# apple/ml-4m

Measured on AMD Instinct MI355X. Metric: multimodal tokens/sec (4M-B train step, whole job), higher is better.
Workload: dtype bf16; 1 GPU; 4M-B mod7 (fm_base_12e_12d_swiglu_nobias, 360.8M params, 8 input / 7 target modalities) masked-modeling train step, 224^2 token grids, 128 input + 128 target tokens/sample, AdamW; model=fm_base_12e_12d_swiglu_nobias, per_gpu_batch=256, global_batch=256, seq_len=256, parallelism=dp1

## Files before the change

### include/fourm_hip.h

```cpp
#ifndef FOURM_HIP_H
#define FOURM_HIP_H
#include <stdint.h>

#ifdef __cplusplus
extern "C" {
#endif

#define FM_ABI_VERSION 11
int fm_abi_version(void);
const char* fm_last_error(void);

enum fm_epilogue {
    FM_EPI_BF16 = 0,
    FM_EPI_GELU = 1,
    FM_EPI_RESIDUAL = 2,
    FM_EPI_SWIGLU = 3,
    FM_EPI_F32 = 4,
    FM_EPI_TANH = 5,
    FM_EPI_SWIGLU_BWD = 6,
    FM_EPI_GELU_BWD = 7,
    FM_EPI_QUICK_GELU = 8,
    FM_EPI_RELU = 9,
    FM_EPI_RELU_BWD = 10
};
// ... 158 lines not shown
} fm_embed_bwd_desc;
int fm_embed_bwd(const fm_embed_bwd_desc* desc, void* stream);

int fm_dense_decoder_mask(const int32_t* cs, const int16_t* mod, void* out, int B, int M, int causal, int use_cs,
                          int use_sep, void* stream);

enum fm_loss_type { FM_LOSS_MOD = 0, FM_LOSS_TOKEN = 1 };
#define FM_SEG_ROWS 256
int fm_segment_rows(const int32_t* head_of_row, int R, int n_heads, int32_t* seg_start, int32_t* seg_count,
                    int32_t* perm, int32_t* row_to_padded, int32_t* tile_group, int Rp, void* stream);
int fm_gather_rows(const void* src, int ld_src, const int32_t* perm, void* dst, int ld_dst, int Rp, int D, void* stream);
int fm_cross_entropy(void* logits, int ldl, const int32_t* perm, const int32_t* tile_group, const int64_t* target_ids,
                     const int32_t* vocab, const int32_t* seg_start, const int32_t* seg_count, const void* grad_scale,
                     int loss_type, int n_heads, int Rp, int max_vocab, void* row_loss, void* row_lse, void* head_loss,
                     void* total_loss, int write_grad, void* stream);

int fm_swiglu_bwd(const void* da, int ldda, const void* gu, int ldgu, void* dgu, int lddgu, int R, int H, int Hp, void* stream);
int fm_gelu_bwd(const void* dh, int lddh, const void* pre, int ldp, void* dpre, int lddp, int R, int H, int Hp, void* stream);
typedef struct fm_shadow_desc {
    const void* src; void* dst;
    int32_t ld_src, ld_dst, rows, cols, transpose, tile_start;
    const void* col_scale;
    int32_t dst_f32, reserved;
} fm_shadow_desc;
int fm_shadow_refresh(const fm_shadow_desc* descs, int n_descs, int total_tiles, void* stream);
#define FM_FOLD_MAX_JOBS 48
typedef struct fm_fold_grad_job {
    const void* dWp; const void* W; const void* gamma; void* gW; void* ggamma;
    int32_t rows, cols, ld_dwp, reserved;
} fm_fold_grad_job;
// ... 223 lines not shown
```

### ml-4m_amd/csrc/loss.hip

```cpp
#include "common.h"
#include "fourm_hip.h"

namespace {

constexpr int SEG_ALIGN = FM_SEG_ROWS;

__global__ __launch_bounds__(1024) void segment_rows_kernel(const int32_t* __restrict__ head_of_row, int R, int n_heads,
                                                            int32_t* __restrict__ seg_start, int32_t* __restrict__ seg_count,
                                                            int32_t* __restrict__ perm, int32_t* __restrict__ row_to_padded,
                                                            int32_t* __restrict__ tile_group, int Rp) {
    __shared__ int cnt[FM_MAX_MODS];
    __shared__ int wtot[16];
    const int g = blockIdx.x, tid = threadIdx.x, lane = tid & 63, wave = tid >> 6;
    if (tid < FM_MAX_MODS) cnt[tid] = 0;
    __syncthreads();
    for (int r = tid; r < R; r += 1024) {
        const int hh = head_of_row[r];
        if (hh >= 0 && hh <= g) atomicAdd(&cnt[hh], 1);
    }
    __syncthreads();
    int start = 0;
    for (int m = 0; m < g; ++m) start += (cnt[m] + SEG_ALIGN - 1) / SEG_ALIGN * SEG_ALIGN;
    const int mine = cnt[g];
    const int padded = (mine + SEG_ALIGN - 1) / SEG_ALIGN * SEG_ALIGN;
// ... 22 lines not shown
        run += tot;
    }
}

__global__ void fill_i32_kernel(int32_t* p, int v, int n) {
    const int i = blockIdx.x * 256 + threadIdx.x;
    if (i < n) p[i] = v;
}

__device__ __forceinline__ void online_merge(float& m, float& s, float m2, float s2) {
    const float mn = fmaxf(m, m2);
    s = s * __expf(m - mn) + s2 * __expf(m2 - mn);
    m = mn;
}

__global__ __launch_bounds__(256) void ce_fwd_kernel(const bf16_t* __restrict__ logits, int ldl, const int32_t* __restrict__ perm,
                                                     const int32_t* __restrict__ tile_group, const long long* __restrict__ target_ids,
                                                     const int32_t* __restrict__ vocab, float* __restrict__ row_loss, float* __restrict__ row_lse) {
    __shared__ float red_m[4], red_s[4];
    const int pr = blockIdx.x;
    const int g = tile_group[pr / SEG_ALIGN];
    if (g < 0) return;
    const int src = perm[pr];
    if (src < 0) {
        if (threadIdx.x == 0) { row_loss[pr] = 0.f; row_lse[pr] = 0.f; }
        return;
    }
    const int V = vocab[g];
    const bf16_t* row = logits + (size_t)pr * ldl;
    float m = -INFINITY, ssum = 0.f;
    for (int c = threadIdx.x * 8; c < V; c += 256 * 8) {
        float v[8];
        if (c + 8 <= V) {
            const uint4 p = *(const uint4*)(row + c);
            const uint32_t w[4] = {p.x, p.y, p.z, p.w};
#pragma unroll
            for (int e = 0; e < 4; ++e) { v[2 * e] = bf2f((bf16_t)(w[e] & 0xffff)); v[2 * e + 1] = bf2f((bf16_t)(w[e] >> 16)); }
        } else {
#pragma unroll
            for (int e = 0; e < 8; ++e) v[e] = c + e < V ? bf2f(row[c + e]) : -INFINITY;
        }
        float cm = v[0];
#pragma unroll
        for (int e = 1; e < 8; ++e) cm = fmaxf(cm, v[e]);
        const float mn = fmaxf(m, cm);
        float add = 0.f;
#pragma unroll
        for (int e = 0; e < 8; ++e) add += __expf(v[e] - mn);
        ssum = ssum * __expf(m - mn) + add;
        m = mn;
    }
#pragma unroll
    for (int o = 32; o > 0; o >>= 1) {
        const float m2 = __shfl_xor(m, o, 64), s2 = __shfl_xor(ssum, o, 64);
        if (m2 > -INFINITY || m > -INFINITY) online_merge(m, ssum, m2, s2);
    }
    const int lane = threadIdx.x & 63, wave = threadIdx.x >> 6;
    if (lane == 0) { red_m[wave] = m; red_s[wave] = ssum; }
    __syncthreads();
    if (threadIdx.x == 0) {
        float M = red_m[0], S = red_s[0];
        for (int w = 1; w < 4; ++w)
            if (red_m[w] > -INFINITY) online_merge(M, S, red_m[w], red_s[w]);
        const float lse = M + __logf(S);
        row_lse[pr] = lse;
        row_loss[pr] = lse - bf2f(row[target_ids[src]]);
    }
}

__global__ __launch_bounds__(256) void ce_bwd_kernel(bf16_t* __restrict__ logits, int ldl, const int32_t* __restrict__ perm,
                                                     const int32_t* __restrict__ tile_group, const long long* __restrict__ target_ids,
                                                     const int32_t* __restrict__ vocab, const int32_t* __restrict__ seg_count,
                                                     const float* __restrict__ gscale, int loss_type, int n_heads,
                                                     const float* __restrict__ row_lse) {
    const int pr = blockIdx.x;
    const int g = tile_group[pr / SEG_ALIGN];
    if (g < 0) return;
    const int V = vocab[g];
    const int Vp = (V + 63) / 64 * 64;
    bf16_t* row = logits + (size_t)pr * ldl;
    const int src = perm[pr];
    if (src < 0) {
        for (int c = threadIdx.x; c < Vp / 8; c += 256) *(uint4*)(row + c * 8) = make_uint4(0u, 0u, 0u, 0u);
        return;
    }
    float w;
    if (loss_type == FM_LOSS_MOD) {
        w = 1.0f / ((float)seg_count[g] * (float)n_heads);
    } else {
        float tot = 0.f;
        for (int mm = 0; mm < n_heads; ++mm) tot += (float)seg_count[mm] * (float)vocab[mm];
        w = (float)V / tot;
    }
    w *= gscale ? gscale[0] : 1.0f;
    const float lse = row_lse[pr];
    const int tgt = (int)target_ids[src];
    for (int c = threadIdx.x * 8; c < Vp; c += 256 * 8) {
        const uint4 p = *(const uint4*)(row + c);
        const uint32_t wd[4] = {p.x, p.y, p.z, p.w};
        float o[8];
#pragma unroll
        for (int e = 0; e < 8; ++e) {
            const float x = bf2f((bf16_t)((e & 1) ? (wd[e >> 1] >> 16) : (wd[e >> 1] & 0xffff)));
            o[e] = (c + e < V) ? (__expf(x - lse) - ((c + e) == tgt ? 1.f : 0.f)) * w : 0.f;
        }
        *(uint4*)(row + c) = make_uint4(pack2bf(o[0], o[1]), pack2bf(o[2], o[3]), pack2bf(o[4], o[5]), pack2bf(o[6], o[7]));
    }
}

__global__ __launch_bounds__(256) void loss_finalize_kernel(const float* __restrict__ row_loss, const int32_t* __restrict__ seg_start,
                                                            const int32_t* __restrict__ seg_count, const int32_t* __restrict__ vocab,
                                                            int n_heads, int loss_type, float* __restrict__ head_loss, float* __restrict__ total) {
    __shared__ float red[4];
    __shared__ float hl[FM_MAX_MODS];
    const int lane = threadIdx.x & 63, wave = threadIdx.x >> 6;
    for (int g = 0; g < n_heads; ++g) {
        const int s0 = seg_start[g], n = seg_count[g];
        float s = 0.f;
        for (int i = threadIdx.x; i < n; i += 256) s += row_loss[s0 + i];
        s = wave_sum(s);
        if (lane == 0) red[wave] = s;
// ... 11 lines not shown
        total[0] = tot / wsum;
    }
}

__global__ __launch_bounds__(256) void ce_f32_kernel(float* logits, int ld, const int* perm, const int* tile_group, const long long* target_ids,
                                                     const int* vocab, const int* seg_count, const float* grad_scale, int loss_type, int n_heads,
                                                     float* row_loss, float* row_lse, int write_grad, int seg_rows) {
    __shared__ float red[4];
    const int pr = blockIdx.x;
    const int g = tile_group[pr / seg_rows];
    if (g < 0) return;
    const int src = perm[pr];
    const int V = vocab[g];
    float* row = logits + (size_t)pr * ld;
    if (src < 0) {
        if (!write_grad) { if (threadIdx.x == 0) { row_loss[pr] = 0.f; row_lse[pr] = 0.f; } }
        else for (int c = threadIdx.x; c < V; c += 256) row[c] = 0.f;
        return;
    }
    const int tgt = (int)target_ids[src];
    if (!write_grad) {
        float mx = -INFINITY;
        for (int c = threadIdx.x; c < V; c += 256) mx = fmaxf(mx, row[c]);
        mx = wave_max(mx);
        __syncthreads();
        if ((threadIdx.x & 63) == 0) red[threadIdx.x >> 6] = mx;
        __syncthreads();
        mx = fmaxf(fmaxf(red[0], red[1]), fmaxf(red[2], red[3]));
        float s = 0.f;
        for (int c = threadIdx.x; c < V; c += 256) s += expf(row[c] - mx);
        s = wave_sum(s);
        __syncthreads();
        if ((threadIdx.x & 63) == 0) red[threadIdx.x >> 6] = s;
        __syncthreads();
        s = (red[0] + red[1]) + (red[2] + red[3]);
        const float lse = mx + logf(s);
        if (threadIdx.x == 0) { row_lse[pr] = lse; row_loss[pr] = lse - row[tgt]; }
        return;
    }
    float coef;
    if (loss_type == FM_LOSS_MOD) coef = 1.0f / ((float)n_heads * (float)seg_count[g]);
    else {
        double tot = 0.0;
        for (int h = 0; h < n_heads; ++h) tot += (double)seg_count[h] * (double)vocab[h];
        coef = (float)((double)V / tot);
    }
    coef *= grad_scale ? grad_scale[0] : 1.0f;
    const float lse = row_lse[pr];
    for (int c = threadIdx.x; c < V; c += 256) row[c] = coef * (expf(row[c] - lse) - (c == tgt ? 1.0f : 0.f));
}


__global__ __launch_bounds__(256) void gather_rows_kernel(const bf16_t* __restrict__ src, int lds_, const int32_t* __restrict__ perm,
                                                          bf16_t* __restrict__ dst, int ldd, int Rp, int D) {
    const int lane = threadIdx.x & 63, wave = threadIdx.x >> 6;
    for (int pr = blockIdx.x * 4 + wave; pr < Rp; pr += gridDim.x * 4) {
        const int s = perm[pr];
        for (int c = lane; c < D / 8; c += 64) {
            uint4 v = make_uint4(0u, 0u, 0u, 0u);
            if (s >= 0) v = *(const uint4*)(src + (size_t)s * lds_ + c * 8);
            *(uint4*)(dst + (size_t)pr * ldd + c * 8) = v;
        }
    }
// ... 20 lines not shown
    if (grid > 4096) grid = 4096;
    hipLaunchKernelGGL(gather_rows_kernel, dim3(grid), dim3(256), 0, (hipStream_t)stream, (const bf16_t*)src, ld_src, perm, (bf16_t*)dst, ld_dst, Rp, D);
    FM_CHECK_LAUNCH("fm_gather_rows");
    return 0;
}

extern "C" int fm_cross_entropy(void* logits, int ldl, const int32_t* perm, const int32_t* tile_group, const int64_t* target_ids,
                                const int32_t* vocab, const int32_t* seg_start, const int32_t* seg_count, const void* grad_scale,
                                int loss_type, int n_heads, int Rp, int max_vocab, void* row_loss, void* row_lse, void* head_loss,
                                void* total_loss, int write_grad, void* stream) {
    FM_CHECK_ARG(logits && perm && tile_group && target_ids && vocab && seg_start && seg_count && row_loss && row_lse && head_loss && total_loss,
                 "fm_cross_entropy: null pointer");
    FM_CHECK_ARG(loss_type == FM_LOSS_MOD || loss_type == FM_LOSS_TOKEN, "fm_cross_entropy: invalid loss type %d", loss_type);
    FM_CHECK_ARG(ldl % 8 == 0 && ldl >= (max_vocab + 63) / 64 * 64, "fm_cross_entropy: ldl=%d too small for vocab %d", ldl, max_vocab);
    FM_CHECK_ARG((((uintptr_t)logits) & 15) == 0, "fm_cross_entropy: logits must be 16-byte aligned");
    if (!write_grad) {
        hipLaunchKernelGGL(ce_fwd_kernel, dim3(Rp), dim3(256), 0, (hipStream_t)stream, (const bf16_t*)logits, ldl, perm, tile_group,
                           (const long long*)target_ids, vocab, (float*)row_loss, (float*)row_lse);
        hipLaunchKernelGGL(loss_finalize_kernel, dim3(1), dim3(256), 0, (hipStream_t)stream, (const float*)row_loss, seg_start, seg_count,
                           vocab, n_heads, loss_type, (float*)head_loss, (float*)total_loss);
    } else {
        hipLaunchKernelGGL(ce_bwd_kernel, dim3(Rp), dim3(256), 0, (hipStream_t)stream, (bf16_t*)logits, ldl, perm, tile_group,
                           (const long long*)target_ids, vocab, seg_count, (const float*)grad_scale, loss_type, n_heads, (const float*)row_lse);
    }
    FM_CHECK_LAUNCH("fm_cross_entropy");
    return 0;
}

extern "C" int fm_cross_entropy_f32(void* logits, int ldl, const int32_t* perm, const int32_t* tile_group, const int64_t* target_ids,
                                    const int32_t* vocab, const int32_t* seg_start, const int32_t* seg_count, const void* grad_scale,
                                    int loss_type, int n_heads, int Rp, int max_vocab, void* row_loss, void* row_lse, void* head_loss,
                                    void* total_loss, int write_grad, void* stream) {
    FM_CHECK_ARG(logits && perm && tile_group && target_ids && vocab && seg_start && seg_count && row_loss && row_lse && head_loss && total_loss,
                 "fm_cross_entropy_f32: null pointer");
    FM_CHECK_ARG(loss_type == FM_LOSS_MOD || loss_type == FM_LOSS_TOKEN, "fm_cross_entropy_f32: invalid loss type %d", loss_type);
    FM_CHECK_ARG(ldl >= max_vocab, "fm_cross_entropy_f32: ldl=%d too small for vocab %d", ldl, max_vocab);
    hipLaunchKernelGGL(ce_f32_kernel, dim3(Rp), dim3(256), 0, (hipStream_t)stream, (float*)logits, ldl, perm, tile_group,
                       (const long long*)target_ids, vocab, seg_count, (const float*)grad_scale, loss_type, n_heads, (float*)row_loss,
                       (float*)row_lse, write_grad, SEG_ALIGN);
    if (!write_grad)
        hipLaunchKernelGGL(loss_finalize_kernel, dim3(1), dim3(256), 0, (hipStream_t)stream, (const float*)row_loss, seg_start, seg_count,
                           vocab, n_heads, loss_type, (float*)head_loss, (float*)total_loss);
    FM_CHECK_LAUNCH("fm_cross_entropy_f32");
    return 0;
}
```

### ml-4m_amd/fourm/hip/_lib.py

```python
import ctypes as C
import os

FM_MAX_MODS = 24
_LIB_PATH = os.environ.get("FOURM_HIP_LIB") or os.path.join(os.path.dirname(os.path.dirname(os.path.abspath(__file__))), "_lib", "libfourm_hip.so")


class FourmHipUnavailable(ImportError):
    pass


def _load():
    if not os.path.exists(_LIB_PATH):
        raise FourmHipUnavailable(
            f"{_LIB_PATH} is missing - build the gfx950 kernels first: python ml-4m_amd/build_ext.py "
            "(the 4M hot path has no fallback implementation)")
    return C.CDLL(_LIB_PATH)


lib = _load()
lib.fm_last_error.restype = C.c_char_p
lib.fm_abi_version.restype = C.c_int
ABI_VERSION = 11
if lib.fm_abi_version() != ABI_VERSION:
    raise FourmHipUnavailable(f"libfourm_hip.so ABI {lib.fm_abi_version()} != expected {ABI_VERSION}; rebuild")
# ... 129 lines not shown
gemm_tn_multi = _sig("fm_gemm_tn_multi", P(GemmTNJob), C.c_int, vp)
layernorm_fwd = _sig("fm_layernorm_fwd", vp, i32, vp, vp, vp, i32, i32, vp, vp, vp, i32, i32, f32, vp)
layernorm_fwd_res = _sig("fm_layernorm_fwd_res", vp, i32, vp, i32, vp, i32, vp, vp, vp, i32, i32, vp, vp, vp, i32, i32, f32, vp)
layernorm_bwd = _sig("fm_layernorm_bwd", vp, i32, vp, vp, i32, vp, vp, vp, vp, vp, i32, vp, i32, vp, vp, i32, i32, vp)
layernorm_bwd_h = _sig("fm_layernorm_bwd_h", vp, i32, vp, i32, vp, i32, vp, vp, vp, vp, vp, i32, vp, i32, vp, i32, i32, vp)
attn_fwd = _sig("fm_attn_fwd", P(AttnArgs), vp)
attn_bwd = _sig("fm_attn_bwd", P(AttnArgs), vp)
attn_decode = _sig("fm_attn_decode", P(AttnDecodeArgs), vp)
ATTN_DECODE_MAX_NK = 8192
select_embed = _sig("fm_select_embed", P(SelectDesc), vp)
embed_bwd = _sig("fm_embed_bwd", P(EmbedBwdDesc), vp)
dense_decoder_mask = _sig("fm_dense_decoder_mask", vp, vp, vp, i32, i32, i32, i32, i32, vp)
segment_rows = _sig("fm_segment_rows", vp, i32, i32, vp, vp, vp, vp, vp, i32, vp)
gather_rows = _sig("fm_gather_rows", vp, i32, vp, vp, i32, i32, i32, vp)
cross_entropy = _sig("fm_cross_entropy", vp, i32, vp, vp, vp, vp, vp, vp, vp, i32, i32, i32, i32, vp, vp, vp, vp, i32, vp)
swiglu_bwd = _sig("fm_swiglu_bwd", vp, i32, vp, i32, vp, i32, i32, i32, i32, vp)
gelu_bwd = _sig("fm_gelu_bwd", vp, i32, vp, i32, vp, i32, i32, i32, i32, vp)
cast_pad = _sig("fm_cast_pad", vp, i32, vp, i32, i32, i32, vp)
transpose_cast_pad = _sig("fm_transpose_cast_pad", vp, i32, vp, i32, i32, i32, i32, vp)
colsum = _sig("fm_colsum", vp, i32, vp, i32, i32, vp)
shadow_refresh = _sig("fm_shadow_refresh", vp, i32, i32, vp)
fold_colscale_grad = _sig("fm_fold_colscale_grad", vp, i32, vp)
headnorm_fwd = _sig("fm_headnorm_fwd", vp, i32, vp, vp, vp, i32, vp, i32, i32, C.c_float, vp)
headnorm_bwd = _sig("fm_headnorm_bwd", vp, i32, vp, i32, vp, vp, vp, i32, vp, vp, i32, i32, vp)
f32_to_bf16 = _sig("fm_f32_to_bf16", vp, vp, i64, vp)
bf16_to_f32_scaled = _sig("fm_bf16_to_f32_scaled", vp, vp, i64, f32, vp)
add_bf16_f32 = _sig("fm_add_bf16_f32", vp, vp, vp, i64, vp)
lib.fm_set_reserved_cus.argtypes = [C.c_int]
lib.fm_get_reserved_cus.restype = C.c_int
lib.fm_get_reserved_cus.argtypes = []
# ... 103 lines not shown
ssim_scale_scratch = _sig("fm_ssim_scale_scratch", i32, i32, i32, i32, i32)
ssim_scale = _sig("fm_ssim_scale", vp, vp, i32, i32, i32, i32, i32, i32, i32, vp, i32, f32, f32, vp, vp, vp, vp)
avgpool2x2_pair = _sig("fm_avgpool2x2_pair", vp, vp, i32, i32, i32, i32, i32, i32, i32, vp, vp, vp)
token_histogram = _sig("fm_token_histogram", vp, i32, i64, i32, vp, vp, vp)
RESIZE_BILINEAR, RESIZE_BILINEAR_AA, RESIZE_NEAREST = 0, 1, 2
RESIZE_MAX_TAPS = 64
resize_axis_table = _sig("fm_resize_axis_table", i32, i32, i32, P(i32), P(i32), P(f32), P(C.c_double), P(i32), P(i32))
resize_bilinear_fwd = _sig("fm_resize_bilinear_fwd", vp, vp, i32, i32, i32, i32, i32, vp, vp, vp, i32, vp, vp, vp, i32, vp, vp, i32, vp)
resize_bilinear_bwd = _sig("fm_resize_bilinear_bwd", vp, vp, i32, i32, i32, i32, i32, vp, vp, vp, i32, vp, vp, vp, vp, vp, i32, vp, vp, vp, i32, vp)
resize_nearest = _sig("fm_resize_nearest", vp, vp, i32, i32, i32, i32, i32, i32, vp, vp, vp)
EXPORTS = ["fm_resize_axis_table", "fm_resize_bilinear_fwd", "fm_resize_bilinear_bwd", "fm_resize_nearest","fm_metric_sums_scratch", "fm_metric_sums", "fm_ssim_scale_scratch", "fm_ssim_scale", "fm_avgpool2x2_pair", "fm_token_histogram",
           "fm_reconst_loss_scratch", "fm_reconst_loss", "fm_scale_f32", "fm_mask_out_samples", "fm_ema_update", "fm_diffusion_pair", "fm_token_usage", "fm_lpips_stem", "fm_lpips_stem_bwd", "fm_maxpool2x2_nhwc", "fm_lpips_distance", "fm_lpips_tap_bwd", "fm_feat_distance", "fm_quick_gelu_bwd", "fm_quick_gelu_bwd_f32", "fm_clip_embed_ln_bwd", "fm_tap_add", "fm_clip_embed_ln", "fm_attn_decode", "fm_vit_patch_rows", "fm_vit_emb_rows", "fm_vit_colsum", "fm_lora_apply", "fm_lora_grad", "fm_vq_assign_wide", "fm_memcodes_assign", "fm_convnext_block", "fm_split3_bf16", "fm_unet_im2col", "fm_groupnorm_nhwc", "fm_add_bf16", "fm_silu_f32_to_bf16", "fm_timestep_embedding", "fm_unet_attention", "fm_diffusion_x0", "fm_quantile_abs",
           "fm_diffusion_step", "fm_unpack_image_u8", "fm_unpack_ids_u16", "fm_unpack_mask_bits", "fm_decoder_attention_from_target", "fm_guidance_combine", "fm_image_mask", "fm_token_budgets", "fm_span_mask", "fm_vq_code_stats", "fm_vq_ema_update", "fm_vq_code_bias", "fm_vq_assign_bias", "fm_vq_code_stats_raw", "fm_vq_ema_update_euclid", "fm_vq_unpatchify", "fm_vq_latent_grad", "fm_tanh_bwd_f32", "fm_embed_rows_f32", "fm_vq_patchify_ex", "fm_vq_cls_emb_bwd", "fm_vq_latent_grad_normalized", "fm_abi_version", "fm_last_error", "fm_gemm_nt", "fm_set_gemm_nt_config", "fm_get_gemm_nt_config", "fm_set_reserved_cus", "fm_get_reserved_cus", "fm_bf16_to_f32_scaled", "fm_add_bf16_f32", "fm_scale_rows_bf16", "fm_gemm_tn", "fm_gemm_tn_multi", "fm_set_gemm_tn_config", "fm_get_gemm_tn_config", "fm_set_tn_transpose_read",
           "fm_get_tn_transpose_read", "fm_layernorm_fwd", "fm_layernorm_fwd_res", "fm_layernorm_bwd", "fm_layernorm_bwd_h", "fm_headnorm_fwd", "fm_headnorm_bwd", "fm_attn_fwd", "fm_attn_bwd",
           "fm_set_attn_transpose_read", "fm_get_attn_transpose_read", "fm_select_embed", "fm_embed_bwd",
           "fm_dense_decoder_mask", "fm_segment_rows", "fm_gather_rows", "fm_cross_entropy", "fm_swiglu_bwd",
           "fm_gelu_bwd", "fm_cast_pad", "fm_transpose_cast_pad", "fm_shadow_refresh", "fm_fold_colscale_grad", "fm_colsum", "fm_f32_to_bf16", "fm_adamw", "fm_adamw_shadow",
           "fm_sumsq", "fm_clip_coef", "fm_vq_patchify", "fm_l2norm_rows", "fm_vq_assign",
           "fm_sample_tokens", "fm_maskgit_commit", "fm_gemm_f32", "fm_attn_f32_fwd", "fm_attn_f32_bwd", "fm_layernorm_bwd_f32", "fm_headnorm_f32_fwd", "fm_headnorm_f32_bwd",
           "fm_swiglu_bwd_f32", "fm_gelu_bwd_f32", "fm_colsum_f32", "fm_cross_entropy_f32", "fm_lab_set",
           "fm_unet_im2col_f32", "fm_groupnorm_nhwc_f32", "fm_unet_attention_f32", "fm_add_f32", "fm_silu_f32", "fm_timestep_embedding_f32",
           "fm_unet_col2im_f32", "fm_groupnorm_nhwc_bwd_f32", "fm_unet_attention_bwd_f32", "fm_silu_bwd_f32"]


def check(rc: int):
    if rc != 0:
        raise RuntimeError(f"libfourm_hip: {lib.fm_last_error().decode()} (rc={rc})")
```

### ml-4m_amd/fourm/hip/engine.py

```python
import math
import os
import random
import weakref
from typing import Dict, List, Optional

import torch
import torch.nn as nn

from . import _lib as L
from . import ops

_WEIGHT_EPOCH = 0
FUSE_ACT_BWD = os.environ.get("FOURM_FUSE_ACT_BWD", "0") == "1"
HEADS_DENSE = os.environ.get("FOURM_HEADS_DENSE", "1") == "1"
HEADS_DENSE_MAX = int(os.environ.get("FOURM_HEADS_DENSE_MAX", "8"))
DEFER_RESIDUAL = os.environ.get("FOURM_DEFER_RESIDUAL", "1") == "1"
HOIST_CTX = os.environ.get("FOURM_HOIST_CTX", "1") == "1"
LN_BWD_FROM_H = os.environ.get("FOURM_LN_BWD_FROM_H", "1") == "1"
DP_RESERVE_ALWAYS = os.environ.get("FOURM_DP_RESERVE_ALWAYS", "0") == "1"


def bump_weight_epoch():
    global _WEIGHT_EPOCH
    _WEIGHT_EPOCH += 1


def ru(x, m):
    return (x + m - 1) // m * m


def is_lora(lin) -> bool:
    return hasattr(lin, "lora_down")

# ... 725 lines not shown
            vt = torch.tensor(vocabs, dtype=i32, device=dev)
            self._head_groups = cache = (key, fwd, bwd, vt)
        hs["g_fwd"], hs["g_bwd"], hs["vocab_t"] = cache[1], cache[2], cache[3]
        logits = ws.get("heads.logits", (Rp, ldl), self.adt)
        if HEADS_DENSE and not self.fp32 and nH <= HEADS_DENSE_MAX and ops.heads_dense_ok(w_fwd, vocabs, logits):
            ops.gemm_nt_heads(yp, w_fwd, vocabs, hs["seg_start"], hs["seg_count"], logits, D)
        else:
            ops.gemm_nt_grouped(yp, hs["g_fwd"], hs["tile_group"], logits, hs["maxV"], max_K=D)
        hs.update(yp=yp, logits=logits, sv=sv)
        hs["row_loss"] = ws.get("heads.row_loss", (Rp,), torch.float32)
        hs["row_lse"] = ws.get("heads.row_lse", (Rp,), torch.float32)
        hs["head_loss"] = ws.get("heads.head_loss", (nH,), torch.float32)
        hs["total"] = ws.get("heads.total", (1,), torch.float32)
        return hs

    def loss_forward(self, dec, hs, loss_type):
        lt = L.LOSS_MOD if loss_type in ("mod", "modality") else L.LOSS_TOKEN
        hs["loss_type"] = lt
        ops.cross_entropy(hs["logits"], hs["perm"], hs["tile_group"], dec["target_ids"].view(-1), hs["vocab_t"], hs["seg_start"],
                          hs["seg_count"], hs["n"], hs["maxV"], hs["row_loss"], hs["row_lse"], hs["head_loss"], hs["total"], loss_type=lt)
        return hs["total"], hs["head_loss"]

    def dec_order(self, mod_dict):
        names = [n for n in mod_dict if n in self.model.decoder_embeddings]
        return random.sample(names, len(names))

    def train_forward(self, mod_dict, n_enc, n_dec, loss_type, save=True):
        if loss_type not in ("mod", "modality", "token"):
            raise ValueError("Invalid loss type")
        self.prepare()
        if save:
            self._ensure_flat()
        enc_names = [n for n in mod_dict if n in self.model.encoder_embeddings]
        enc = self.select(mod_dict, n_enc, False, enc_names, "enc.")
        dec = self.select(mod_dict, n_dec, True, self.dec_order(mod_dict), "dec.")
        y, st = self.trunk_forward(enc, dec, save)
        hs = self.heads_setup(dec, y, save)
        total, head_loss = self.loss_forward(dec, hs, loss_type)
        if save:
            self._ctx = dict(enc=enc, dec=dec, st=st, hs=hs)
        return total, head_loss, hs["heads"], hs["seg_count"]

    def _g(self, p):
        return self.grad_view(p) if p.requires_grad else None

    def _dW(self, dy, x, lin, R64, n_cols=None, dy_cols=None):
        g = self._g(lin.weight)
        N = lin.weight.shape[0] if n_cols is None else n_cols
        if g is not None:
            if self._dw_jobs is not None:
                self._dw_jobs.append((dy, x, g.view(g.shape[0], -1), N, lin.weight[0].numel(), R64))
            else:
                ops.gemm_tn(dy, x, g.view(g.shape[0], -1), N=N, K=lin.weight[0].numel(), R=R64)
# ... 177 lines not shown
    def train_backward(self, grad_scale: torch.Tensor):
        c = self._ctx
        if c is None:
            raise RuntimeError("train_backward without a preceding training forward")
        self._ctx, self._dw_jobs = None, None
        if self.reducer is not None:
            self.reducer.begin()
            if getattr(self.reducer, "reserved_cus", 0):
                L.lib.fm_set_reserved_cus(int(self.reducer.reserved_cus))
        m, ws = self.model, self.ws
        enc, dec, st, hs = c["enc"], c["dec"], c["st"], c["hs"]
        B, N, Mt, D = enc["B"], enc["Nt"], dec["Nt"], self.D
        bf, f32 = self.adt, torch.float32
        Rq, Rc = B * Mt, B * N
        Rqp, Rcp = st["y_final"].shape[0], st["x_final"].shape[0]
        ops.cross_entropy(hs["logits"], hs["perm"], hs["tile_group"], dec["target_ids"].view(-1), hs["vocab_t"], hs["seg_start"],
                          hs["seg_count"], hs["n"], hs["maxV"], hs["row_loss"], hs["row_lse"], hs["head_loss"], hs["total"],
                          loss_type=hs["loss_type"], grad_scale=grad_scale, write_grad=True)
        dyp = ws.get("bwd.dyp", (hs["Rp"], D), bf)
        ops.gemm_nt_grouped(hs["logits"], hs["g_bwd"], hs["tile_group"], dyp, D, max_K=ru(hs["maxV"], 64))
        heads = [m.decoder_embeddings[h] for h in hs["heads"]]
        if any(h.to_logits.weight.requires_grad for h in heads):
            outs = [self.grad_view(h.to_logits.weight) if h.to_logits.weight.requires_grad else None for h in heads]
            key = tuple(o.data_ptr() if o is not None else 0 for o in outs)
            cache = getattr(self, "_head_tn_groups", None)
            if cache is None or cache[0] != key:
                cache = self._head_tn_groups = (key, ops.make_groups(
                    [dict(out=o, N=(v if o is not None else 0)) for o, v in zip(outs, hs["vocabs"])], self.device))
            tn = cache[1]
            ops.gemm_tn_grouped(hs["logits"], hs["yp"], tn, hs["seg_start"], hs["seg_count"], hs["n"], hs["maxV"], hs["Rp"], D)
        g = ws.get("bwd.g_dec", (Rqp, D), f32)
        g_bf = ws.get("bwd.g_dec_bf", (Rqp, D), bf)
        self._ln_bwd(m.decoder_norm, dyp, st["y_final"], hs["sv"], "dn", g, g_bf, Rq, dres=None, dy_row_map=hs["r2p"])
# ... 61 lines not shown
```

### ml-4m_amd/fourm/hip/ops.py

```python
import contextlib
import ctypes as C
import threading
from typing import Optional

import torch

from . import _lib as L

_PROFILER = None


def set_profiler(p):
    global _PROFILER
    _PROFILER = p


class _Null:
    def __enter__(self):
        return self

    def __exit__(self, *a):
        return False


# ... 353 lines not shown
    L.check(L.segment_rows(_p(head_of_row), head_of_row.numel(), n_heads, _p(seg_start), _p(seg_count), _p(perm),
                           _p(row_to_padded), _p(tile_group), perm.numel(), _stream()))


@_timed("heads_misc")
def gather_rows(src, perm, dst, D):
    L.check(L.gather_rows(_p(src), _ld(src), _p(perm), _p(dst), _ld(dst), perm.numel(), D, _stream()))


@_timed("cross_entropy")
def cross_entropy(logits, perm, tile_group, target_ids, vocab, seg_start, seg_count, n_heads, max_vocab, row_loss, row_lse, head_loss,
                  total_loss, *, loss_type=L.LOSS_MOD, grad_scale=None, write_grad=False):
    fn = L.cross_entropy_f32 if logits.dtype == torch.float32 else L.cross_entropy
    L.check(fn(_p(logits), _ld(logits), _p(perm), _p(tile_group), _p(target_ids), _p(vocab), _p(seg_start),
                            _p(seg_count), _p(grad_scale), loss_type, n_heads, perm.numel(), max_vocab, _p(row_loss), _p(row_lse),
                            _p(head_loss), _p(total_loss), 1 if write_grad else 0, _stream()))


@_timed("swiglu_bwd")
def swiglu_bwd(da, gu, dgu, H, Hp, R=None):
    if da.dtype == torch.float32:
        return L.check(L.swiglu_bwd_f32(_p(da), _ld(da), _p(gu), _ld(gu), _p(dgu), _ld(dgu), da.shape[0] if R is None else R, H, Hp, _stream()))
    L.check(L.swiglu_bwd(_p(da), _ld(da), _p(gu), _ld(gu), _p(dgu), _ld(dgu), da.shape[0] if R is None else R, H, Hp, _stream()))


@_timed("gelu_bwd")
def gelu_bwd(dh, pre, dpre, H, Hp, R=None):
    if dh.dtype == torch.float32:
        return L.check(L.gelu_bwd_f32(_p(dh), _ld(dh), _p(pre), _ld(pre), _p(dpre), _ld(dpre), dh.shape[0] if R is None else R, H, _stream()))
    L.check(L.gelu_bwd(_p(dh), _ld(dh), _p(pre), _ld(pre), _p(dpre), _ld(dpre), dh.shape[0] if R is None else R, H, Hp, _stream()))

# ... 433 lines not shown
```

Measured before the change: 1.159 million tokens/s.

## Fuse cross-entropy forward and gradient into one pass over logits

Adds a one-pass cross-entropy kernel that keeps each row's logits in registers, computes the log-sum-exp and loss, then overwrites the logits in place with the unscaled gradient during the forward pass. Backward then only launches a rescale kernel, which returns early when the grad scale is 1. This removes a second full read of the large logits buffer and one kernel launch per step. In exchange the logits are destroyed at forward time, and register pressure rises with the templated chunk counts.

```diff
diff --git a/include/fourm_hip.h b/include/fourm_hip.h
--- a/include/fourm_hip.h
+++ b/include/fourm_hip.h
@@ -196,6 +196,8 @@
                      const int32_t* vocab, const int32_t* seg_start, const int32_t* seg_count, const void* grad_scale,
                      int loss_type, int n_heads, int Rp, int max_vocab, void* row_loss, void* row_lse, void* head_loss,
                      void* total_loss, int write_grad, void* stream);
+int fm_cross_entropy_rescale(void* dlogits, int ldl, const int32_t* tile_group, const int32_t* vocab, const void* grad_scale, int Rp,
+                             int max_vocab, int is_f32, void* stream);
 
 int fm_swiglu_bwd(const void* da, int ldda, const void* gu, int ldgu, void* dgu, int lddgu, int R, int H, int Hp, void* stream);
 int fm_gelu_bwd(const void* dh, int lddh, const void* pre, int ldp, void* dpre, int lddp, int R, int H, int Hp, void* stream);
diff --git a/ml-4m_amd/csrc/loss.hip b/ml-4m_amd/csrc/loss.hip
--- a/ml-4m_amd/csrc/loss.hip
+++ b/ml-4m_amd/csrc/loss.hip
@@ -60,6 +60,47 @@
     m = mn;
 }
 
+__device__ __forceinline__ void ce_decode8(const uint4 p, int c, int V, float v[8]) {
+    const uint32_t w[4] = {p.x, p.y, p.z, p.w};
+#pragma unroll
+    for (int e = 0; e < 4; ++e) { v[2 * e] = bf2f((bf16_t)(w[e] & 0xffff)); v[2 * e + 1] = bf2f((bf16_t)(w[e] >> 16)); }
+    if (c + 8 > V) {
+#pragma unroll
+        for (int e = 0; e < 8; ++e) if (c + e >= V) v[e] = -INFINITY;
+    }
+}
+
+__device__ __forceinline__ void ce_accum8(const float v[8], float& m, float& ssum) {
+    float cm = v[0];
+#pragma unroll
+    for (int e = 1; e < 8; ++e) cm = fmaxf(cm, v[e]);
+    const float mn = fmaxf(m, cm);
+    float add = 0.f;
+#pragma unroll
+    for (int e = 0; e < 8; ++e) add += __expf(v[e] - mn);
+    ssum = ssum * __expf(m - mn) + add;
+    m = mn;
+}
+
+__device__ __forceinline__ float ce_block_lse(float m, float ssum, float* red_m, float* red_s) {
+#pragma unroll
+    for (int o = 32; o > 0; o >>= 1) {
+        const float m2 = __shfl_xor(m, o, 64), s2 = __shfl_xor(ssum, o, 64);
+        if (m2 > -INFINITY || m > -INFINITY) online_merge(m, ssum, m2, s2);
+    }
+    const int lane = threadIdx.x & 63, wave = threadIdx.x >> 6;
+    if (lane == 0) { red_m[wave] = m; red_s[wave] = ssum; }
+    __syncthreads();
+    float lse = 0.f;
+    if (threadIdx.x == 0) {
+        float M = red_m[0], S = red_s[0];
+        for (int w = 1; w < 4; ++w)
+            if (red_m[w] > -INFINITY) online_merge(M, S, red_m[w], red_s[w]);
+        lse = M + __logf(S);
+    }
+    return lse;
+}
+
 __global__ __launch_bounds__(256) void ce_fwd_kernel(const bf16_t* __restrict__ logits, int ldl, const int32_t* __restrict__ perm,
                                                      const int32_t* __restrict__ tile_group, const long long* __restrict__ target_ids,
                                                      const int32_t* __restrict__ vocab, float* __restrict__ row_loss, float* __restrict__ row_lse) {
@@ -77,41 +118,33 @@
     float m = -INFINITY, ssum = 0.f;
     for (int c = threadIdx.x * 8; c < V; c += 256 * 8) {
         float v[8];
-        if (c + 8 <= V) {
-            const uint4 p = *(const uint4*)(row + c);
-            const uint32_t w[4] = {p.x, p.y, p.z, p.w};
-#pragma unroll
-            for (int e = 0; e < 4; ++e) { v[2 * e] = bf2f((bf16_t)(w[e] & 0xffff)); v[2 * e + 1] = bf2f((bf16_t)(w[e] >> 16)); }
-        } else {
-#pragma unroll
-            for (int e = 0; e < 8; ++e) v[e] = c + e < V ? bf2f(row[c + e]) : -INFINITY;
-        }
-        float cm = v[0];
-#pragma unroll
-        for (int e = 1; e < 8; ++e) cm = fmaxf(cm, v[e]);
-        const float mn = fmaxf(m, cm);
-        float add = 0.f;
-#pragma unroll
-        for (int e = 0; e < 8; ++e) add += __expf(v[e] - mn);
-        ssum = ssum * __expf(m - mn) + add;
-        m = mn;
-    }
-#pragma unroll
-    for (int o = 32; o > 0; o >>= 1) {
-        const float m2 = __shfl_xor(m, o, 64), s2 = __shfl_xor(ssum, o, 64);
-        if (m2 > -INFINITY || m > -INFINITY) online_merge(m, ssum, m2, s2);
-    }
-    const int lane = threadIdx.x & 63, wave = threadIdx.x >> 6;
-    if (lane == 0) { red_m[wave] = m; red_s[wave] = ssum; }
-    __syncthreads();
+        ce_decode8(*(const uint4*)(row + c), c, V, v);
+        ce_accum8(v, m, ssum);
+    }
+    const float lse = ce_block_lse(m, ssum, red_m, red_s);
     if (threadIdx.x == 0) {
-        float M = red_m[0], S = red_s[0];
-        for (int w = 1; w < 4; ++w)
-            if (red_m[w] > -INFINITY) online_merge(M, S, red_m[w], red_s[w]);
-        const float lse = M + __logf(S);
         row_lse[pr] = lse;
         row_loss[pr] = lse - bf2f(row[target_ids[src]]);
     }
+}
+
+__device__ __forceinline__ float ce_head_weight(int g, int V, const int32_t* __restrict__ vocab, const int32_t* __restrict__ seg_count,
+                                                int loss_type, int n_heads) {
+    if (loss_type == FM_LOSS_MOD) return 1.0f / ((float)seg_count[g] * (float)n_heads);
+    float tot = 0.f;
+    for (int mm = 0; mm < n_heads; ++mm) tot += (float)seg_count[mm] * (float)vocab[mm];
+    return (float)V / tot;
+}
+
+__device__ __forceinline__ uint4 ce_grad8(const uint4 p, int c, int V, int tgt, float lse, float w) {
+    const uint32_t wd[4] = {p.x, p.y, p.z, p.w};
+    float o[8];
+#pragma unroll
+    for (int e = 0; e < 8; ++e) {
+        const float x = bf2f((bf16_t)((e & 1) ? (wd[e >> 1] >> 16) : (wd[e >> 1] & 0xffff)));
+        o[e] = (c + e < V) ? (__expf(x - lse) - ((c + e) == tgt ? 1.f : 0.f)) * w : 0.f;
+    }
+    return make_uint4(pack2bf(o[0], o[1]), pack2bf(o[2], o[3]), pack2bf(o[4], o[5]), pack2bf(o[6], o[7]));
 }
 
 __global__ __launch_bounds__(256) void ce_bwd_kernel(bf16_t* __restrict__ logits, int ldl, const int32_t* __restrict__ perm,
@@ -130,27 +163,101 @@
         for (int c = threadIdx.x; c < Vp / 8; c += 256) *(uint4*)(row + c * 8) = make_uint4(0u, 0u, 0u, 0u);
         return;
     }
-    float w;
-    if (loss_type == FM_LOSS_MOD) {
-        w = 1.0f / ((float)seg_count[g] * (float)n_heads);
-    } else {
-        float tot = 0.f;
-        for (int mm = 0; mm < n_heads; ++mm) tot += (float)seg_count[mm] * (float)vocab[mm];
-        w = (float)V / tot;
-    }
+    float w = ce_head_weight(g, V, vocab, seg_count, loss_type, n_heads);
     w *= gscale ? gscale[0] : 1.0f;
     const float lse = row_lse[pr];
     const int tgt = (int)target_ids[src];
-    for (int c = threadIdx.x * 8; c < Vp; c += 256 * 8) {
-        const uint4 p = *(const uint4*)(row + c);
-        const uint32_t wd[4] = {p.x, p.y, p.z, p.w};
-        float o[8];
-#pragma unroll
-        for (int e = 0; e < 8; ++e) {
-            const float x = bf2f((bf16_t)((e & 1) ? (wd[e >> 1] >> 16) : (wd[e >> 1] & 0xffff)));
-            o[e] = (c + e < V) ? (__expf(x - lse) - ((c + e) == tgt ? 1.f : 0.f)) * w : 0.f;
-        }
-        *(uint4*)(row + c) = make_uint4(pack2bf(o[0], o[1]), pack2bf(o[2], o[3]), pack2bf(o[4], o[5]), pack2bf(o[6], o[7]));
+    for (int c = threadIdx.x * 8; c < Vp; c += 256 * 8) *(uint4*)(row + c) = ce_grad8(*(const uint4*)(row + c), c, V, tgt, lse, w);
+}
+
+template <int NCH>
+__global__ __launch_bounds__(256) void ce_onepass_kernel(bf16_t* __restrict__ logits, int ldl, const int32_t* __restrict__ perm,
+                                                         const int32_t* __restrict__ tile_group, const long long* __restrict__ target_ids,
+                                                         const int32_t* __restrict__ vocab, const int32_t* __restrict__ seg_count, int loss_type,
+                                                         int n_heads, float* __restrict__ row_loss, float* __restrict__ row_lse) {
+    __shared__ float red_m[4], red_s[4], lse_sh;
+    const int pr = blockIdx.x;
+    const int g = tile_group[pr / SEG_ALIGN];
+    if (g < 0) return;
+    const int V = vocab[g];
+    const int Vp = (V + 63) / 64 * 64;
+    bf16_t* row = logits + (size_t)pr * ldl;
+    const int src = perm[pr];
+    if (src < 0) {
+        if (threadIdx.x == 0) { row_loss[pr] = 0.f; row_lse[pr] = 0.f; }
+        for (int c = threadIdx.x; c < Vp / 8; c += 256) *(uint4*)(row + c * 8) = make_uint4(0u, 0u, 0u, 0u);
+        return;
+    }
+    uint4 keep[NCH > 0 ? NCH : 1];
+    float m = -INFINITY, ssum = 0.f;
+    if constexpr (NCH > 0) {
+#pragma unroll
+        for (int k = 0; k < NCH; ++k) {
+            const int c = (k * 256 + threadIdx.x) * 8;
+            keep[k] = *(const uint4*)(row + (c < V ? c : 0));
+        }
+#pragma unroll
+        for (int k = 0; k < NCH; ++k) {
+            const int c = (k * 256 + threadIdx.x) * 8;
+            asm volatile("" : "+v"(keep[k].x), "+v"(keep[k].y), "+v"(keep[k].z), "+v"(keep[k].w));
+            if (c < V) {
+                float v[8];
+                ce_decode8(keep[k], c, V, v);
+                ce_accum8(v, m, ssum);
+            }
+        }
+    } else {
+        for (int c = threadIdx.x * 8; c < V; c += 256 * 8) {
+            float v[8];
+            ce_decode8(*(const uint4*)(row + c), c, V, v);
+            ce_accum8(v, m, ssum);
+        }
+    }
+    const int tgt = (int)target_ids[src];
+    float lse = ce_block_lse(m, ssum, red_m, red_s);
+    if (threadIdx.x == 0) {
+        row_lse[pr] = lse;
+        row_loss[pr] = lse - bf2f(row[tgt]);
+        lse_sh = lse;
+    }
+    __syncthreads();
+    lse = lse_sh;
+    const float w = ce_head_weight(g, V, vocab, seg_count, loss_type, n_heads);
+    if constexpr (NCH > 0) {
+#pragma unroll
+        for (int k = 0; k < NCH; ++k) {
+            const int c = (k * 256 + threadIdx.x) * 8;
+            asm volatile("" : "+v"(keep[k].x), "+v"(keep[k].y), "+v"(keep[k].z), "+v"(keep[k].w));
+            if (c < Vp) *(uint4*)(row + c) = ce_grad8(keep[k], c, V, tgt, lse, w);
+        }
+    } else {
+        for (int c = threadIdx.x * 8; c < Vp; c += 256 * 8) *(uint4*)(row + c) = ce_grad8(*(const uint4*)(row + c), c, V, tgt, lse, w);
+    }
+}
+
+template <typename T>
+__global__ __launch_bounds__(256) void ce_rescale_kernel(T* __restrict__ logits, int ldl, const int32_t* __restrict__ tile_group,
+                                                         const int32_t* __restrict__ vocab, const float* __restrict__ gscale, int Rp) {
+    const float s = gscale[0];
+    if (s == 1.0f) return;
+    for (int pr = blockIdx.x; pr < Rp; pr += gridDim.x) {
+        const int g = tile_group[pr / SEG_ALIGN];
+        if (g < 0) continue;
+        const int V = vocab[g];
+        T* row = logits + (size_t)pr * ldl;
+        if constexpr (sizeof(T) == 2) {
+            const int Vp = (V + 63) / 64 * 64;
+            for (int c = threadIdx.x * 8; c < Vp; c += 256 * 8) {
+                const uint4 p = *(const uint4*)(row + c);
+                const uint32_t wd[4] = {p.x, p.y, p.z, p.w};
+                uint32_t o[4];
+#pragma unroll
+                for (int e = 0; e < 4; ++e) o[e] = pack2bf(bf2f((bf16_t)(wd[e] & 0xffff)) * s, bf2f((bf16_t)(wd[e] >> 16)) * s);
+                *(uint4*)(row + c) = make_uint4(o[0], o[1], o[2], o[3]);
+            }
+        } else {
+            for (int c = threadIdx.x; c < V; c += 256) row[c] *= s;
+        }
     }
 }
 
@@ -192,12 +299,13 @@
     const int V = vocab[g];
     float* row = logits + (size_t)pr * ld;
     if (src < 0) {
-        if (!write_grad) { if (threadIdx.x == 0) { row_loss[pr] = 0.f; row_lse[pr] = 0.f; } }
-        else for (int c = threadIdx.x; c < V; c += 256) row[c] = 0.f;
+        if (write_grad != 1) { if (threadIdx.x == 0) { row_loss[pr] = 0.f; row_lse[pr] = 0.f; } }
+        if (write_grad) for (int c = threadIdx.x; c < V; c += 256) row[c] = 0.f;
         return;
     }
     const int tgt = (int)target_ids[src];
-    if (!write_grad) {
+    float lse;
+    if (write_grad != 1) {
         float mx = -INFINITY;
         for (int c = threadIdx.x; c < V; c += 256) mx = fmaxf(mx, row[c]);
         mx = wave_max(mx);
@@ -212,9 +320,12 @@
         if ((threadIdx.x & 63) == 0) red[threadIdx.x >> 6] = s;
         __syncthreads();
         s = (red[0] + red[1]) + (red[2] + red[3]);
-        const float lse = mx + logf(s);
+        lse = mx + logf(s);
         if (threadIdx.x == 0) { row_lse[pr] = lse; row_loss[pr] = lse - row[tgt]; }
-        return;
+        if (!write_grad) return;
+        __syncthreads();
+    } else {
+        lse = row_lse[pr];
     }
     float coef;
     if (loss_type == FM_LOSS_MOD) coef = 1.0f / ((float)n_heads * (float)seg_count[g]);
@@ -223,8 +334,7 @@
         for (int h = 0; h < n_heads; ++h) tot += (double)seg_count[h] * (double)vocab[h];
         coef = (float)((double)V / tot);
     }
-    coef *= grad_scale ? grad_scale[0] : 1.0f;
-    const float lse = row_lse[pr];
+    if (write_grad == 1) coef *= grad_scale ? grad_scale[0] : 1.0f;
     for (int c = threadIdx.x; c < V; c += 256) row[c] = coef * (expf(row[c] - lse) - (c == tgt ? 1.0f : 0.f));
 }
 
@@ -275,7 +385,20 @@
     FM_CHECK_ARG(loss_type == FM_LOSS_MOD || loss_type == FM_LOSS_TOKEN, "fm_cross_entropy: invalid loss type %d", loss_type);
     FM_CHECK_ARG(ldl % 8 == 0 && ldl >= (max_vocab + 63) / 64 * 64, "fm_cross_entropy: ldl=%d too small for vocab %d", ldl, max_vocab);
     FM_CHECK_ARG((((uintptr_t)logits) & 15) == 0, "fm_cross_entropy: logits must be 16-byte aligned");
-    if (!write_grad) {
+    FM_CHECK_ARG(write_grad >= 0 && write_grad <= 2, "fm_cross_entropy: invalid write_grad %d", write_grad);
+    if (write_grad == 2) {
+        const int chunks = ((max_vocab + 63) / 64 * 64 + 2047) / 2048;
+#define FM_CE_ONEPASS(NCH)                                                                                                              \
+    hipLaunchKernelGGL(ce_onepass_kernel<NCH>, dim3(Rp), dim3(256), 0, (hipStream_t)stream, (bf16_t*)logits, ldl, perm, tile_group,     \
+                       (const long long*)target_ids, vocab, seg_count, loss_type, n_heads, (float*)row_loss, (float*)row_lse)
+        if (chunks <= 4) FM_CE_ONEPASS(4);
+        else if (chunks <= 8) FM_CE_ONEPASS(8);
+        else if (chunks <= 15) FM_CE_ONEPASS(15);
+        else FM_CE_ONEPASS(0);
+#undef FM_CE_ONEPASS
+        hipLaunchKernelGGL(loss_finalize_kernel, dim3(1), dim3(256), 0, (hipStream_t)stream, (const float*)row_loss, seg_start, seg_count,
+                           vocab, n_heads, loss_type, (float*)head_loss, (float*)total_loss);
+    } else if (!write_grad) {
         hipLaunchKernelGGL(ce_fwd_kernel, dim3(Rp), dim3(256), 0, (hipStream_t)stream, (const bf16_t*)logits, ldl, perm, tile_group,
                            (const long long*)target_ids, vocab, (float*)row_loss, (float*)row_lse);
         hipLaunchKernelGGL(loss_finalize_kernel, dim3(1), dim3(256), 0, (hipStream_t)stream, (const float*)row_loss, seg_start, seg_count,
@@ -296,12 +419,32 @@
                  "fm_cross_entropy_f32: null pointer");
     FM_CHECK_ARG(loss_type == FM_LOSS_MOD || loss_type == FM_LOSS_TOKEN, "fm_cross_entropy_f32: invalid loss type %d", loss_type);
     FM_CHECK_ARG(ldl >= max_vocab, "fm_cross_entropy_f32: ldl=%d too small for vocab %d", ldl, max_vocab);
+    FM_CHECK_ARG(write_grad >= 0 && write_grad <= 2, "fm_cross_entropy_f32: invalid write_grad %d", write_grad);
     hipLaunchKernelGGL(ce_f32_kernel, dim3(Rp), dim3(256), 0, (hipStream_t)stream, (float*)logits, ldl, perm, tile_group,
                        (const long long*)target_ids, vocab, seg_count, (const float*)grad_scale, loss_type, n_heads, (float*)row_loss,
                        (float*)row_lse, write_grad, SEG_ALIGN);
-    if (!write_grad)
+    if (write_grad != 1)
         hipLaunchKernelGGL(loss_finalize_kernel, dim3(1), dim3(256), 0, (hipStream_t)stream, (const float*)row_loss, seg_start, seg_count,
                            vocab, n_heads, loss_type, (float*)head_loss, (float*)total_loss);
     FM_CHECK_LAUNCH("fm_cross_entropy_f32");
     return 0;
 }
+
+extern "C" int fm_cross_entropy_rescale(void* dlogits, int ldl, const int32_t* tile_group, const int32_t* vocab, const void* grad_scale, int Rp,
+                                        int max_vocab, int is_f32, void* stream) {
+    FM_CHECK_ARG(dlogits && tile_group && vocab && grad_scale, "fm_cross_entropy_rescale: null pointer");
+    FM_CHECK_ARG(Rp > 0 && Rp % SEG_ALIGN == 0, "fm_cross_entropy_rescale: Rp=%d is no multiple of %d", Rp, SEG_ALIGN);
+    const int grid = Rp < 4096 ? Rp : 4096;
+    if (is_f32) {
+        FM_CHECK_ARG(ldl >= max_vocab, "fm_cross_entropy_rescale: ldl=%d too small for vocab %d", ldl, max_vocab);
+        hipLaunchKernelGGL(ce_rescale_kernel<float>, dim3(grid), dim3(256), 0, (hipStream_t)stream, (float*)dlogits, ldl, tile_group, vocab,
+                           (const float*)grad_scale, Rp);
+    } else {
+        FM_CHECK_ARG(ldl % 8 == 0 && ldl >= (max_vocab + 63) / 64 * 64, "fm_cross_entropy_rescale: ldl=%d too small for vocab %d", ldl, max_vocab);
+        FM_CHECK_ARG((((uintptr_t)dlogits) & 15) == 0, "fm_cross_entropy_rescale: d(logits) must be 16-byte aligned");
+        hipLaunchKernelGGL(ce_rescale_kernel<bf16_t>, dim3(grid), dim3(256), 0, (hipStream_t)stream, (bf16_t*)dlogits, ldl, tile_group, vocab,
+                           (const float*)grad_scale, Rp);
+    }
+    FM_CHECK_LAUNCH("fm_cross_entropy_rescale");
+    return 0;
+}
diff --git a/ml-4m_amd/fourm/hip/_lib.py b/ml-4m_amd/fourm/hip/_lib.py
--- a/ml-4m_amd/fourm/hip/_lib.py
+++ b/ml-4m_amd/fourm/hip/_lib.py
@@ -167,6 +167,7 @@
 segment_rows = _sig("fm_segment_rows", vp, i32, i32, vp, vp, vp, vp, vp, i32, vp)
 gather_rows = _sig("fm_gather_rows", vp, i32, vp, vp, i32, i32, i32, vp)
 cross_entropy = _sig("fm_cross_entropy", vp, i32, vp, vp, vp, vp, vp, vp, vp, i32, i32, i32, i32, vp, vp, vp, vp, i32, vp)
+cross_entropy_rescale = _sig("fm_cross_entropy_rescale", vp, i32, vp, vp, vp, i32, i32, i32, vp)
 swiglu_bwd = _sig("fm_swiglu_bwd", vp, i32, vp, i32, vp, i32, i32, i32, i32, vp)
 gelu_bwd = _sig("fm_gelu_bwd", vp, i32, vp, i32, vp, i32, i32, i32, i32, vp)
 cast_pad = _sig("fm_cast_pad", vp, i32, vp, i32, i32, i32, vp)
@@ -300,7 +301,7 @@
            "fm_diffusion_step", "fm_unpack_image_u8", "fm_unpack_ids_u16", "fm_unpack_mask_bits", "fm_decoder_attention_from_target", "fm_guidance_combine", "fm_image_mask", "fm_token_budgets", "fm_span_mask", "fm_vq_code_stats", "fm_vq_ema_update", "fm_vq_code_bias", "fm_vq_assign_bias", "fm_vq_code_stats_raw", "fm_vq_ema_update_euclid", "fm_vq_unpatchify", "fm_vq_latent_grad", "fm_tanh_bwd_f32", "fm_embed_rows_f32", "fm_vq_patchify_ex", "fm_vq_cls_emb_bwd", "fm_vq_latent_grad_normalized", "fm_abi_version", "fm_last_error", "fm_gemm_nt", "fm_set_gemm_nt_config", "fm_get_gemm_nt_config", "fm_set_reserved_cus", "fm_get_reserved_cus", "fm_bf16_to_f32_scaled", "fm_add_bf16_f32", "fm_scale_rows_bf16", "fm_gemm_tn", "fm_gemm_tn_multi", "fm_set_gemm_tn_config", "fm_get_gemm_tn_config", "fm_set_tn_transpose_read",
            "fm_get_tn_transpose_read", "fm_layernorm_fwd", "fm_layernorm_fwd_res", "fm_layernorm_bwd", "fm_layernorm_bwd_h", "fm_headnorm_fwd", "fm_headnorm_bwd", "fm_attn_fwd", "fm_attn_bwd",
            "fm_set_attn_transpose_read", "fm_get_attn_transpose_read", "fm_select_embed", "fm_embed_bwd",
-           "fm_dense_decoder_mask", "fm_segment_rows", "fm_gather_rows", "fm_cross_entropy", "fm_swiglu_bwd",
+           "fm_dense_decoder_mask", "fm_segment_rows", "fm_gather_rows", "fm_cross_entropy", "fm_cross_entropy_rescale", "fm_swiglu_bwd",
            "fm_gelu_bwd", "fm_cast_pad", "fm_transpose_cast_pad", "fm_shadow_refresh", "fm_fold_colscale_grad", "fm_colsum", "fm_f32_to_bf16", "fm_adamw", "fm_adamw_shadow",
            "fm_sumsq", "fm_clip_coef", "fm_vq_patchify", "fm_l2norm_rows", "fm_vq_assign",
            "fm_sample_tokens", "fm_maskgit_commit", "fm_gemm_f32", "fm_attn_f32_fwd", "fm_attn_f32_bwd", "fm_layernorm_bwd_f32", "fm_headnorm_f32_fwd", "fm_headnorm_f32_bwd",
diff --git a/ml-4m_amd/fourm/hip/engine.py b/ml-4m_amd/fourm/hip/engine.py
--- a/ml-4m_amd/fourm/hip/engine.py
+++ b/ml-4m_amd/fourm/hip/engine.py
@@ -17,6 +17,7 @@
 DEFER_RESIDUAL = os.environ.get("FOURM_DEFER_RESIDUAL", "1") == "1"
 HOIST_CTX = os.environ.get("FOURM_HOIST_CTX", "1") == "1"
 LN_BWD_FROM_H = os.environ.get("FOURM_LN_BWD_FROM_H", "1") == "1"
+CE_ONEPASS = os.environ.get("FOURM_CE_ONEPASS", "1") == "1"
 DP_RESERVE_ALWAYS = os.environ.get("FOURM_DP_RESERVE_ALWAYS", "0") == "1"
 
 
@@ -772,11 +773,12 @@
         hs["total"] = ws.get("heads.total", (1,), torch.float32)
         return hs
 
-    def loss_forward(self, dec, hs, loss_type):
+    def loss_forward(self, dec, hs, loss_type, with_grad=False):
         lt = L.LOSS_MOD if loss_type in ("mod", "modality") else L.LOSS_TOKEN
-        hs["loss_type"] = lt
+        hs["loss_type"], hs["grad_written"] = lt, with_grad
         ops.cross_entropy(hs["logits"], hs["perm"], hs["tile_group"], dec["target_ids"].view(-1), hs["vocab_t"], hs["seg_start"],
-                          hs["seg_count"], hs["n"], hs["maxV"], hs["row_loss"], hs["row_lse"], hs["head_loss"], hs["total"], loss_type=lt)
+                          hs["seg_count"], hs["n"], hs["maxV"], hs["row_loss"], hs["row_lse"], hs["head_loss"], hs["total"], loss_type=lt,
+                          write_grad=2 if with_grad else 0)
         return hs["total"], hs["head_loss"]
 
     def dec_order(self, mod_dict):
@@ -794,7 +796,7 @@
         dec = self.select(mod_dict, n_dec, True, self.dec_order(mod_dict), "dec.")
         y, st = self.trunk_forward(enc, dec, save)
         hs = self.heads_setup(dec, y, save)
-        total, head_loss = self.loss_forward(dec, hs, loss_type)
+        total, head_loss = self.loss_forward(dec, hs, loss_type, with_grad=save and CE_ONEPASS)
         if save:
             self._ctx = dict(enc=enc, dec=dec, st=st, hs=hs)
         return total, head_loss, hs["heads"], hs["seg_count"]
@@ -1002,9 +1004,12 @@
         bf, f32 = self.adt, torch.float32
         Rq, Rc = B * Mt, B * N
         Rqp, Rcp = st["y_final"].shape[0], st["x_final"].shape[0]
-        ops.cross_entropy(hs["logits"], hs["perm"], hs["tile_group"], dec["target_ids"].view(-1), hs["vocab_t"], hs["seg_start"],
-                          hs["seg_count"], hs["n"], hs["maxV"], hs["row_loss"], hs["row_lse"], hs["head_loss"], hs["total"],
-                          loss_type=hs["loss_type"], grad_scale=grad_scale, write_grad=True)
+        if hs["grad_written"]:
+            ops.cross_entropy_rescale(hs["logits"], hs["tile_group"], hs["vocab_t"], hs["maxV"], grad_scale)
+        else:
+            ops.cross_entropy(hs["logits"], hs["perm"], hs["tile_group"], dec["target_ids"].view(-1), hs["vocab_t"], hs["seg_start"],
+                              hs["seg_count"], hs["n"], hs["maxV"], hs["row_loss"], hs["row_lse"], hs["head_loss"], hs["total"],
+                              loss_type=hs["loss_type"], grad_scale=grad_scale, write_grad=True)
         dyp = ws.get("bwd.dyp", (hs["Rp"], D), bf)
         ops.gemm_nt_grouped(hs["logits"], hs["g_bwd"], hs["tile_group"], dyp, D, max_K=ru(hs["maxV"], 64))
         heads = [m.decoder_embeddings[h] for h in hs["heads"]]
diff --git a/ml-4m_amd/fourm/hip/ops.py b/ml-4m_amd/fourm/hip/ops.py
--- a/ml-4m_amd/fourm/hip/ops.py
+++ b/ml-4m_amd/fourm/hip/ops.py
@@ -391,7 +391,13 @@
     fn = L.cross_entropy_f32 if logits.dtype == torch.float32 else L.cross_entropy
     L.check(fn(_p(logits), _ld(logits), _p(perm), _p(tile_group), _p(target_ids), _p(vocab), _p(seg_start),
                             _p(seg_count), _p(grad_scale), loss_type, n_heads, perm.numel(), max_vocab, _p(row_loss), _p(row_lse),
-                            _p(head_loss), _p(total_loss), 1 if write_grad else 0, _stream()))
+                            _p(head_loss), _p(total_loss), int(write_grad), _stream()))
+
+
+@_timed("cross_entropy")
+def cross_entropy_rescale(dlogits, tile_group, vocab, max_vocab, grad_scale):
+    L.check(L.cross_entropy_rescale(_p(dlogits), _ld(dlogits), _p(tile_group), _p(vocab), _p(grad_scale), dlogits.shape[0], max_vocab,
+                                    1 if dlogits.dtype == torch.float32 else 0, _stream()))
 
 
 @_timed("swiglu_bwd")
```

New measurement: 1.163 million tokens/s (median of 6 runs). Within noise of the previous version (+0.4%).
